# ryanelandt/PressureFieldContact.jl

Measured on AMD Instinct MI355X. Metric: tet-tri clip+integrate ops/s, higher is better.
Workload: dtype f64

## Files before the change

### pressurefieldcontact.jl_amd/csrc/pfc_bp.h

```cpp
#pragma once

struct BpArgs {
    const ItemRec *items;
    const WorkRec *fin;
    WorkRec *fout;
    WorkRec *cand;
    int *fcount;
    int *ccount;
    int *icnt;
    unsigned *status;
    int level, fcap, ccap;
    int n_items;
};

__device__ __forceinline__ void count_per_item(int *icnt, int item, int slot, bool listed, bool flag, int n = 1) {
    if (__ballot(flag) == 0) return;
    const Seg sg = seg_setup(listed ? item : -1);
    const int t = seg_sum(flag ? n : 0, sg);
    if (sg.tail && sg.valid && t != 0) atomicAdd(&icnt[4 * (size_t)item + slot], t);
}

__device__ __forceinline__ NodeRec load_node(const NodeRec *n) {
    union U { vec4i v[9]; NodeRec r; __device__ U() {} } u;
    const gvec4i *p = (const gvec4i *)n;
// ... 185 lines not shown
        if (valid && sub < 9) {
            const int i = sub % 3, jj = sub / 3;
            const double r0 = na->R[3 * i], r1 = na->R[3 * i + 1], r2 = na->R[3 * i + 2];
            T[i + 3 * jj] = (r0 * pose[3 * jj] + r1 * pose[3 * jj + 1]) + r2 * pose[3 * jj + 2];
        } else if (valid && sub < 12) {
            const int i = sub - 9;
            const double r0 = na->R[3 * i], r1 = na->R[3 * i + 1], r2 = na->R[3 * i + 2];
            const double nt = ((-r0) * na->c[0] + (-r1) * na->c[1]) + (-r2) * na->c[2];
            tt[i] = ((r0 * pose[9] + r1 * pose[10]) + r2 * pose[11]) + nt;
        }
        __syncthreads();
        if (valid && sub < 9) {
            const int i = sub % 3, jj = sub / 3;
            const double r = (T[i] * nb->R[3 * jj] + T[i + 3] * nb->R[3 * jj + 1]) + T[i + 6] * nb->R[3 * jj + 2];
            R[i + 3 * jj] = r;
            aR[i + 3 * jj] = __builtin_fabs(r) + 1.0e-14;
        } else if (valid && sub < 12) {
            const int i = sub - 9;
            t[i] = ((T[i] * nb->c[0] + T[i + 3] * nb->c[1]) + T[i + 6] * nb->c[2]) + tt[i];
        }
        __syncthreads();
        bool sep = false;
        if (valid && sub < 15) {
#define EA_(i) (na->e[(i)])
#define EB_(i) (nb->e[(i)])
#define R_(i, j) R[(i) + 3 * (j)]
#define AR_(i, j) aR[(i) + 3 * (j)]
            if (sub < 3) {
                const int i = sub;
                const double rb = (AR_(i, 0) * EB_(0) + AR_(i, 1) * EB_(1)) + AR_(i, 2) * EB_(2);
                sep = (EA_(i) + rb) < __builtin_fabs(t[i]);
            } else if (sub < 6) {
                const int jj = sub - 3;
                const double tl = __builtin_fabs((R_(0, jj) * t[0] + R_(1, jj) * t[1]) + R_(2, jj) * t[2]);
                const double ra = (AR_(0, jj) * EA_(0) + AR_(1, jj) * EA_(1)) + AR_(2, jj) * EA_(2);
                sep = (ra + EB_(jj)) < tl;
            } else {
                const int m = (sub - 6) / 3, jj = (sub - 6) % 3;
                const int u = (m + 1) % 3, v = (m + 2) % 3;
                const int p100 = jj == 0 ? 1 : 0, p221 = jj == 2 ? 1 : 2;
                const double tl = __builtin_fabs(t[v] * R_(u, jj) - t[u] * R_(v, jj));
                const double ra = EA_(u) * AR_(v, jj) + EA_(v) * AR_(u, jj);
                const double rb = EB_(p100) * AR_(m, p221) + EB_(p221) * AR_(m, p100);
                sep = (ra + rb) < tl;
            }
#undef EA_
#undef EB_
#undef R_
#undef AR_
        }
        const unsigned long long ms = __ballot(sep);
        if (valid && sub == 0) und_v[j] = ((ms >> ((tid & 63) & ~15)) & 0xFFFFull) ? 0 : 1;
        __syncthreads();
    }
}


__device__ __forceinline__ int next_ticket_block(int *ctr, int *slot, int n_seed) {
    if ((int)gridDim.x >= n_seed) return n_seed;
    if (threadIdx.x == 0) *slot = (int)gridDim.x + atomicAdd(ctr, 1);
    __syncthreads();
    const int t = *slot;
    __syncthreads();
    return t;
}

template <int BLK>
__device__ __forceinline__ void flush_candidates(const Dfs32Args &g, const int2 *ob, int n_out, int item, int tid,
                                                 int *s_base) {
    if (tid == 0) *s_base = atomicAdd(g.ccount, n_out);
    __syncthreads();
    const int base = *s_base;
    for (int j = tid; j < n_out; j += BLK) {
        if (base + j < g.ccap) {
            WorkRec c;
            c.item = item; c.a = ob[j].x; c.b = ob[j].y; c.pad = 0;
            g.cand[base + j] = c;
        }
    }
    if (tid == 0 && base + n_out > g.ccap) atomicOr(g.status, kStCandOvf);
    __syncthreads();
}

template <int BLK>
__global__ void __launch_bounds__(BLK, 4) k_bp_dfs32(Dfs32Args g) {
    constexpr int kWaves = BLK / 64, kStack = BLK * 10, kOut = BLK * 5;
    __shared__ int2 stk[kStack];
    __shared__ int2 ob[kOut];
    __shared__ int s_cnt[kWaves][2];
    __shared__ int2 und_l[BLK];
    __shared__ int und_v[BLK];
    __shared__ double xs[(BLK / 16) * 33];
    __shared__ int s_seed, s_base, s_def[2];
    __shared__ double s_pose[12];
    __shared__ float s_q12[4];
    __shared__ float s_posef[13];
    __shared__ int s_pose_exact;
    const int tid = threadIdx.x, lane = tid & 63, wave = tid >> 6;
    int n_seed = *g.n_seed;
    if (n_seed > g.seed_cap) n_seed = g.seed_cap;
    const vec4i s_first = ((const gvec4i *)g.seeds)[blockIdx.x];
    for (int sd = blockIdx.x; sd < n_seed; sd = next_ticket_block(g.next_seed, &s_seed, n_seed)) {
        vec4i s_v = s_first;
        if (sd != (int)blockIdx.x) s_v = ((const gvec4i *)g.seeds)[__builtin_amdgcn_readfirstlane(sd)];
        WorkRec s;
        s.item = s_v.x; s.a = s_v.y; s.b = s_v.z; s.pad = s_v.w;
        if ((unsigned)s.item >= (unsigned)g.n_items) {
            if (tid == 0) atomicOr(g.status, kStHole);
            continue;
        }
        const int item = __builtin_amdgcn_readfirstlane(s.item);
        const ItemRec *it = g.items + item;
        if (tid < 9) { const double x = it->R12[tid]; s_pose[tid] = x; s_posef[tid] = (float)x; }
        else if (tid < 12) { const double x = it->t12[tid - 9]; s_pose[tid] = x; s_posef[tid] = (float)x; }
        else if (tid < 16) s_q12[tid - 12] = it->q12[tid - 12];
        else if (tid == 16) s_pose_exact = it->pose_exact;
        else if (tid == 17) s_posef[12] = it->bp_eabs;
        const NodeF *n1 = it->nf1, *n2 = it->nf2;
        int sp = 1, n_out = 0, n_test = 0, n_cand = 0, n_def = 0, n_und = 0;
        if (tid == 0) {
            const int sa = (s.pad & 1) ? ~s.a : s.a;
            const int sb = (s.pad & 2) ? ~s.b : s.b;
            stk[0] = make_int2(sa, sb);
            s_def[0] = s_def[1] = 0;
        }
        __syncthreads();
#ifdef PFC_STAMPS
        unsigned long long c_a = 0, c_b = 0, c_c = 0, c_d = 0, c_it = 0, c_p = 0, c_w1 = 0, c_w2 = 0;
#endif
        int par = 0;
        for (int guard = 0; (sp > 0 || n_def > 0) && guard < (1 << 22); ++guard, par ^= 1) {
            unsigned long long u0 = 0, u1 = 0, u2 = 0, u3 = 0, u4 = 0; (void)u0; (void)u1; (void)u2; (void)u3; (void)u4;
            STAMP(u0);
            const bool settle = n_def > 0;
            int pw = (kStack - g.reserve - sp) / 3;
            int p = sp < BLK ? sp : BLK;
            if (pw < 1) pw = 1;
            if (p > pw) p = pw;
            if (settle) {
                p = n_def;
                exact_pairs_coop<BLK>(it->nodes1, it->nodes2, s_pose, und_l, n_def, xs, und_v, tid);
            }
            const bool act = tid < p;
            int2 e = make_int2(0, 0);
            if (act) e = settle ? und_l[tid] : stk[sp - 1 - tid];
            if (!settle) { sp -= p; n_test += p; } else { n_und += p; }
            int verdict = 0, a0 = 0, a1 = 0, b0 = 0, b1 = 0;
            if (settle && act) verdict = und_v[tid];
            const bool la = act && e.x < 0, lb = act && e.y < 0;
            if (act) {
                const NodeF a = load_nodef(n1 + node_index(e.x));
                const NodeF b = load_nodef(n2 + node_index(e.y));
                a0 = a.link0; a1 = a.link1; b0 = b.link0; b1 = b.link1;
#ifdef PFC_STAMPS
                { float keep = a.e[0] + b.e[0] + a.q[3] + b.q[3]; asm volatile("" ::"v"(keep)); }
                STAMP(u1);
#endif
                if (!settle) {
                    float R12[9], t12[3], q12[4];
#pragma unroll
                    for (int k = 0; k < 9; ++k) R12[k] = s_posef[k];
#pragma unroll
                    for (int k = 0; k < 3; ++k) t12[k] = s_posef[9 + k];
#pragma unroll
                    for (int k = 0; k < 4; ++k) q12[k] = s_q12[k];
                    __builtin_amdgcn_s_setprio(0);
                    verdict = test_pair_f32(a, b, la || lb, R12, q12, t12, s_posef[12]);
                    __builtin_amdgcn_s_setprio(1);
                    if (s_pose_exact) verdict = 2;
                }
            }
            STAMP(u2);
            if (verdict == 2) und_l[atomicAdd(&s_def[par], 1)] = e;
            const bool hit = verdict == 1;
            const bool is_cand = hit && la && lb;
            const bool two = hit && (la != lb);
            const bool four = hit && !la && !lb;
            const unsigned long long mc = __ballot(is_cand), m2 = __ballot(two), m4 = __ballot(four);
            if (lane == 0) {
                s_cnt[wave][0] = __builtin_popcountll(mc);
                s_cnt[wave][1] = 2 * __builtin_popcountll(m2) + 4 * __builtin_popcountll(m4);
            }
#ifdef PFC_STAMPS
            const unsigned long long w1a = __builtin_amdgcn_s_memtime();
#endif
            __syncthreads();
#ifdef PFC_STAMPS
            c_w1 += __builtin_amdgcn_s_memtime() - w1a;
#endif
            STAMP(u3);
            n_def = s_def[par];
            if (tid == 0) s_def[par ^ 1] = 0;
            int c_off = 0, p_off = 0, c_tot = 0, p_tot = 0;
#pragma unroll
            for (int w = 0; w < kWaves; ++w) {
                const int c = s_cnt[w][0], q = s_cnt[w][1];
                if (w < wave) { c_off += c; p_off += q; }
                c_tot += c; p_tot += q;
            }
            if (is_cand) ob[n_out + c_off + prefix_count(mc)] = make_int2(a0, b0);
            if (two | four) {
                const int pos = sp + p_off + 2 * prefix_count(m2) + 4 * prefix_count(m4);
                if (two) {
                    if (la) {
                        stk[pos] = make_int2(e.x, b0); stk[pos + 1] = make_int2(e.x, b1);
                    } else {
                        stk[pos] = make_int2(a0, e.y); stk[pos + 1] = make_int2(a1, e.y);
                    }
                } else {
                    stk[pos] = make_int2(a0, b0); stk[pos + 1] = make_int2(a1, b0);
                    stk[pos + 2] = make_int2(a0, b1); stk[pos + 3] = make_int2(a1, b1);
                }
            }
            n_out += c_tot;
            sp += p_tot;
#ifdef PFC_STAMPS
            const unsigned long long w2a = __builtin_amdgcn_s_memtime();
#endif
            __syncthreads();
#ifdef PFC_STAMPS
            c_w2 += __builtin_amdgcn_s_memtime() - w2a;
#endif
            if (n_out > kOut - BLK || (sp == 0 && n_def == 0 && n_out > 0)) {
                flush_candidates<BLK>(g, ob, n_out, item, tid, &s_base);
                n_cand += n_out;
                n_out = 0;
            }
#ifdef PFC_STAMPS
            STAMP(u4);
            if (!settle) {
                c_a += u1 - u0; c_b += u2 - u1; c_c += u3 - u2; c_d += u4 - u3; c_it += 1; c_p += (unsigned long long)p;
            }
#endif
        }
#ifdef PFC_STAMPS
        if (lane == 0 && g.stamps) { atomicAdd(&g.stamps[0], c_w1); atomicAdd(&g.stamps[1], c_w2); atomicAdd(&g.stamps[2], c_it); }
        if (tid == 0 && g.stamps) {
            atomicAdd(&g.stamps[8], c_a); atomicAdd(&g.stamps[9], c_b); atomicAdd(&g.stamps[10], c_c);
            atomicAdd(&g.stamps[13], c_d); atomicAdd(&g.stamps[11], c_it); atomicAdd(&g.stamps[12], c_p);
        }
#endif
        if (tid == 0) {
            if (sp > 0 || n_def > 0) atomicOr(g.status, kStAbort);
            atomicAdd(&g.icnt[4 * (size_t)item], n_test);
            if (n_cand) atomicAdd(&g.icnt[4 * (size_t)item + 1], n_cand);
            if (n_und) atomicAdd(g.ucount, n_und);
        }
    }
}

struct NodeHead {
    double c[3], e[3];
    int child0, child1, leaf, aabb;
};
__device__ __forceinline__ NodeHead load_head(const NodeRec *n) {
    union { vec4i v[4]; NodeHead h; } u;
    const gvec4i *p = (const gvec4i *)n;
    u.v[0] = p[0]; u.v[1] = p[1]; u.v[2] = p[2]; u.v[3] = p[3];
    return u.h;
}

__global__ void __launch_bounds__(64) k_bp_dfs(DfsArgs g) {
    __shared__ int2 stk[kDfsStack];
    __shared__ int2 ob[kDfsOut];
    const int lane = threadIdx.x;
    int n_seed = *g.n_seed;
    if (n_seed > g.seed_cap) n_seed = g.seed_cap;
    for (int sd = next_ticket(g.next_seed); sd < n_seed; sd = next_ticket(g.next_seed)) {
        const WorkRec s = g.seeds[sd];
        if ((unsigned)s.item >= (unsigned)g.n_items) {
            if (lane == 0) atomicOr(g.status, kStHole);
            continue;
        }
        const int item = __builtin_amdgcn_readfirstlane(s.item);
        const ItemRec *it = g.items + item;
        double R12[9], aR12[9], t12[3];
#pragma unroll
        for (int k = 0; k < 9; ++k) { R12[k] = it->R12[k]; aR12[k] = __builtin_fabs(R12[k]) + 1.0e-14; }
#pragma unroll
        for (int k = 0; k < 3; ++k) t12[k] = it->t12[k];
        const NodeRec *n1 = it->nodes1, *n2 = it->nodes2;
        int sp = 1, n_out = 0, n_test = 0, n_cand = 0;
        if (lane == 0) {
            const int sa = (((const GNodeRec *)n1)[s.a].leaf != kInternal) ? ~s.a : s.a;
            const int sb = (((const GNodeRec *)n2)[s.b].leaf != kInternal) ? ~s.b : s.b;
            stk[0] = make_int2(sa, sb);
        }
        __syncthreads();
#ifdef PFC_STAMPS
        unsigned long long c_load = 0, c_sat = 0, c_push = 0, c_iter = 0, c_lanes = 0;
#endif
        for (int guard = 0; sp > 0 && guard < (1 << 22); ++guard) {
            unsigned long long u0 = 0, u1 = 0, u2 = 0, u3 = 0;
            (void)u0; (void)u1; (void)u2; (void)u3;
            STAMP(u0);
            int pw = (kDfsStack - g.reserve - sp) / 3;
            int p = sp < 64 ? sp : 64;
            if (pw < 1) pw = 1;
            if (p > pw) p = pw;
            const bool act = lane < p;
            int2 e = make_int2(0, 0);
            if (act) e = stk[sp - 1 - lane];
            __syncthreads();
            sp -= p;
            n_test += p;
            const bool la = act && e.x < 0, lb = act && e.y < 0;
            const int ia = node_index(e.x), ib = node_index(e.y);
            NodeHead a, b;
            a.leaf = kInternal; b.leaf = kInternal; a.child0 = a.child1 = b.child0 = b.child1 = 0; a.aabb = b.aabb = 1;
#pragma unroll
            for (int k = 0; k < 3; ++k) { a.c[k] = a.e[k] = b.c[k] = b.e[k] = 0.0; }
            double Ra[9] = {1.0, 0.0, 0.0, 0.0, 1.0, 0.0, 0.0, 0.0, 1.0}, Rb[9] = {1.0, 0.0, 0.0, 0.0, 1.0, 0.0, 0.0, 0.0, 1.0};
            if (act) {
                a = load_head(n1 + ia);
                b = load_head(n2 + ib);
            }
            const bool ra = la || (act && !a.aabb), rb = lb || (act && !b.aabb);
            const bool general = __any(ra || rb);
            if (ra) {
#pragma unroll
                for (int k = 0; k < 9; ++k) Ra[k] = ((const GNodeRec *)n1)[ia].R[k];
            }
// ... 95 lines not shown
```

### pressurefieldcontact.jl_amd/csrc/pfc_hip.hip

```cpp
#include "pfc_kernels.h"

#include <algorithm>
#include <atomic>
#include <chrono>
#include <condition_variable>
#include <functional>
#include <mutex>
#include <thread>
#include <cmath>
#include <cstdlib>
#include <limits>
#include <cstdarg>
#include <cstdio>
#include <cstring>
#include <string>
#include <utility>
#include <vector>

#include "../../include/pfc.h"
#include "pfc_sort.h"

namespace pfc {

__global__ void k_prep_tri(int n, const double *__restrict__ pt, const int *__restrict__ tri, TriRec *__restrict__ out) {
// ... 247 lines not shown
    template <class T> int out(T *host, size_t count) { return add(Out, host, count); }
    template <class T> int scratch(size_t count) { return add(0, (const T *)nullptr, count); }
    hipError_t commit() {
        hipError_t e = nf > kMaxFields ? hipErrorInvalidValue : buf.ensure(total);
        for (int k = 0; k < nf && e == hipSuccess; ++k)
            if ((f[k].dir & In) && f[k].host && f[k].count)
                e = hipMemcpyAsync(buf.p + f[k].off, f[k].host, f[k].elem * f[k].count, hipMemcpyHostToDevice, st);
        return e;
    }
    template <class T> T *at(int k) const { return f[k].host || !f[k].dir ? reinterpret_cast<T *>(buf.p + f[k].off) : nullptr; }
    hipError_t fetch(int k, size_t count) {
        if (!f[k].host || !count) return hipSuccess;
        return hipMemcpyAsync(f[k].host, buf.p + f[k].off, f[k].elem * count, hipMemcpyDeviceToHost, st);
    }
    hipError_t finish() {
        hipError_t e = hipSuccess;
        for (int k = 0; k < nf && e == hipSuccess; ++k)
            if (f[k].dir & Out) e = fetch(k, f[k].count);
        return e == hipSuccess ? hipStreamSynchronize(st) : e;
    }
};

struct KinHost {
    int n_body = 0, nq = 0, nv = 0;
    std::vector<char> blob;
    size_t o_jtype = 0, o_qoff = 0, o_voff = 0, o_path_off = 0, o_path = 0, o_x_p_j = 0, o_axis = 0, o_anc = 0;
    size_t o_sub_off = 0, o_sub = 0, o_inertia = 0;
    bool has_inertia = false;
    double gravity[3] = {0.0, 0.0, 0.0};
    template <class T> size_t put(const std::vector<T> &v) {
        const size_t off = blob.size(), bytes = sizeof(T) * v.size();
        blob.resize((off + bytes + 255) & ~(size_t)255);
        if (bytes) std::memcpy(blob.data() + off, v.data(), bytes);
        return off;
    }
};

struct HostMesh {
    int n_pt = 0, n_tri = 0, n_tet = 0, n_node = 0, n_leaf = 0, depth = 0;
    double Ebar = 0.0;
    std::vector<double> xyz, eps;
    std::vector<int> tri, tet;
    std::vector<NodeRec> nodes;
    std::vector<NodeF> nodesf;
    double cmax = 0.0;
    NodeRec *d_nodes = nullptr;
    NodeF *d_nodesf = nullptr;
    TriRec *d_tri = nullptr;
    TetRec *d_tet = nullptr;
    double *d_tet_eps = nullptr;
};

enum { EV_START = 0, EV_SETUP, EV_BP, EV_NP, EV_BR, EV_FIN, EV_COUNT };

}

struct pfc_multi;
struct pfc_context {
    int device = 0;
    bool finalized = false;
    pfc_multi *multi = nullptr;
    Stream stream;
    Stream twin_stream;
    PinBuf<char, 2> pin_bp;
    int pin_bp_n = 0;
    bool team_owner = false;
    int opt_team_fault = -1;
    int opt_dual_fold = 1;
    int opt_fused_f32 = 1;
    std::string err;
    std::vector<HostMesh> meshes;
    std::vector<InsDev> ins;
    MeshDev *d_meshes = nullptr;
    InsDev *d_ins = nullptr;
    InsFull *d_insfull = nullptr;
    DevBuf<MeshDev> own_meshes;
    DevBuf<InsDev> own_ins;
    DevBuf<InsFull> own_insfull;
    DevBuf<char> mesh_arena;
    int max_levels = 1;
    int max_leaves = 2;
    bool any_bristle = false, any_tet_tet = false;
    int opt_debug = 0, opt_profile = 0, opt_max_levels = 0, opt_bfs_levels = -1, opt_no_filter = 0;
    DevBuf<ItemRec> items;
    DevBuf<WorkRec> frontier[2], cand;
    DevBuf<int> clip_n, icnt, trac_item;
    DevBuf<double> acc, res, trac_d, rec;
    DevBuf<int> ctr;
    DevBuf<unsigned> status;
    DevBuf<unsigned long long> stamps;
    DevBuf<int> tail;
    PinBuf<int> h_tail;
    PinBuf<char, 2> pin_in, pin_out;
    DevBuf<char> bar_in;
    DevBuf<char> bar_din;
    int bar_state = 0;
    PinBuf<char, 2> pin_din, pin_dout;
    long long dual_hint = -1;
    int dual_dev_hyb_skip = 0;
    struct KeptPass {
        enum Kind { None, Batched, HandOver, Hybrid, OneGraph } kind = None;
        int n = 0;
        bool ids = false;
    } kept;
    bool device_kept() const { return kept.kind == KeptPass::Batched || kept.kind == KeptPass::HandOver; }
    struct Pending {
        enum Kind { None, Batched, Fused, More, Surface } kind = None;
        hipStream_t stream = nullptr;
        int split_n0 = 0, n_ctr = 0;
        enum Dual { NoDual, DualBatched, DualHandOver } dual = NoDual;
        int n_dir = 0; size_t dpcap = 0; bool ids = false;
    } pend;
    struct HostPoint {
        int n = 0;
        bool ids = false;
        unsigned long long serial = 0;
        size_t ids_at = 0;
    };
    HostPoint pin_in_pt;
    HostPoint pin_din_pt;
    bool last_dual_reused = false;
    int opt_dual_reuse = 1;
    unsigned long long value_serial = 0;
    std::vector<int> dual_counts_cache;
    DevBuf<double> dual_zero;
    unsigned long long epoch = 0;
    GraphExec gexec[2];
    struct GraphKey {
        int n_items, levels, L, debug, bristle, surv;
        const void *p[9];
        void *stream;
        unsigned long long epoch;
    } gkey[2] = {};
    bool ghave[2] = {false, false};
    GraphExec dgexec;
    struct DualGraphKey { GraphKey v; int n_dir; size_t bound; const void *din, *dout; } dgkey = {};
    bool dghave = false;
    int opt_graph = 1;
    size_t fcap = 0, ccap = 0, tcap = 0, rcap = 0;
    DevBuf<double> h_pose;
    int last_n_items = 0, last_levels = 0, last_bfs_levels = 0;
    long long stats[8] = {0, 0, 0, 0, 0, 0, 0, 0};
    DevBuf<double> dual_in, dual_acc, dual_res, dual_out, dual_poly;
    DevBuf<int2> dual_pkey;
    DevBuf<int> dual_sel, dual_flag;
    DevBuf<char> stage;
    DevBuf<double> sdual_w;
    DevBuf<int> sdual_i;
    DevBuf<char> sdual_tmp;
    DevBuf<int> surv;
    DevBuf<int> rgn;
    DevBuf<int> poly_item, pcnt, poly_cand;
    DevBuf<double> poly;
    long long last_undecided = 0;
    long long last_active = 0;
    struct ShapeHint { int n = 0; bool sparse = false; } hints[4];
    void note_shape(int n, bool sparse) {
        int k = 0;
        while (k < 3 && hints[k].n != n) ++k;
        for (; k > 0; --k) hints[k] = hints[k - 1];
        hints[0].n = n; hints[0].sparse = sparse;
    }
    bool shape_is_sparse(int n) const {
        for (const ShapeHint &e : hints) if (e.n == n) return e.sparse;
        return false;
    }
// ... 236 lines not shown
    if ((e = ensure_graphed(h, h->tail, (size_t)h->max_levels + 40)) != hipSuccess) return e;
    if ((e = h->h_tail.ensure((size_t)h->max_levels + 40)) != hipSuccess) return e;
    if (h->opt_poison) {
        if ((e = hipMemsetAsync(h->frontier[0].p, 0xFF, sizeof(WorkRec) * h->frontier[0].cap, h->stream)) != hipSuccess) return e;
        if ((e = hipMemsetAsync(h->frontier[1].p, 0xFF, sizeof(WorkRec) * h->frontier[1].cap, h->stream)) != hipSuccess) return e;
        if ((e = hipMemsetAsync(h->cand.p, 0xFF, sizeof(WorkRec) * h->cand.cap, h->stream)) != hipSuccess) return e;
        if (h->poly_item.p && (e = hipMemsetAsync(h->poly_item.p, 0xFF, sizeof(int) * h->poly_item.cap, h->stream)) != hipSuccess) return e;
        if ((e = hipStreamSynchronize(h->stream)) != hipSuccess) return e;
    }
    return hipSuccess;
}

TracSoA trac_view(pfc_context *h) {
    TracSoA t;
    size_t n = h->tcap;
    double *d = h->trac_d.p;
    t.item = h->trac_item.p;
    t.nx = d; t.ny = d + n; t.nz = d + 2 * n; t.rx = d + 3 * n; t.ry = d + 4 * n; t.rz = d + 5 * n;
    t.dA = d + 6 * n; t.p = d + 7 * n;
    return t;
}

int eff_levels(const pfc_context *h) {
    return (h->opt_max_levels > 0 && h->opt_max_levels < h->max_levels) ? h->opt_max_levels : h->max_levels;
}

constexpr int kDualSelectMin = 512;
constexpr int kBpSmallBlockMin = 3072;

int bfs_levels_for(const pfc_context *h, int n_items, int levels, bool half) {
    int L = 0;
    if (h->opt_bfs_levels >= 0) {
        L = h->opt_bfs_levels;
    } else {
        const bool big = h->max_leaves >= 8192, mid = h->max_leaves >= 1024;
        const int n_eff = half ? 2 * n_items : n_items;
        const double target = big ? (n_eff >= 600 ? 1.0 : (n_eff >= 256 ? 1024.0 : (n_eff >= 128 ? 2048.0 : (n_eff >= 32 ? 16384.0 : 49152.0))))
                                  : (mid ? 256.0 : 64.0);
        double seeds = (double)n_items;
        while (seeds < target && L < 9) { seeds *= 4.0; ++L; }
    }
    return L > levels ? levels : L;
}

bool pile_mode(const pfc_context *h, int n_items) {
    return h->max_leaves < 8192 && n_items >= 1024 && n_items < kBpSmallBlockMin && h->shape_is_sparse(n_items) && !h->is_twin;
}

int bp_block_for(const pfc_context *h, int n_items, bool half) {
    if (n_items >= kBpSmallBlockMin) return 128;
    if (half) return 256;
    if (h->max_leaves >= 8192 && n_items >= 8 && n_items < 1024) return 512;
    if (pile_mode(h, n_items)) return 512;
    return 256;
}

void launch_broadphase(pfc_context *h, int n_items, int L, bool half, int *ccount, int *fcount, int *next_seed, int *ucount, hipStream_t st) {
    for (int lv = 0; lv < L; ++lv) {
        BpArgs b;
        b.items = h->items.p; b.fin = h->frontier[lv & 1].p; b.fout = h->frontier[(lv + 1) & 1].p;
        b.cand = h->cand.p; b.fcount = fcount; b.ccount = ccount; b.icnt = h->icnt.p; b.status = h->status.p;
        b.level = lv; b.fcap = (int)h->fcap; b.ccap = (int)h->ccap; b.n_items = n_items;
        double ub = (double)n_items * std::pow(4.0, (double)(lv < 15 ? lv : 15));
        size_t bound = ub > (double)h->fcap ? h->fcap : (size_t)ub;
        hipLaunchKernelGGL(k_bp_expand, dim3(grid_for(bound, 256, 2048)), dim3(256), 0, st, b);
    }
    {
        double ub = (double)n_items * std::pow(4.0, (double)(L < 15 ? L : 15));
        size_t bound = ub > (double)h->fcap ? h->fcap : (size_t)ub;
        DfsArgs d;
        d.items = h->items.p; d.cand = h->cand.p; d.ccount = ccount; d.ccap = (int)h->ccap; d.icnt = h->icnt.p;
        d.status = h->status.p; d.reserve = 3 * h->max_levels + 3; d.stamps = h->stamps.p; d.n_items = n_items;
        if (h->opt_no_filter) {
            d.seeds = h->frontier[L & 1].p; d.n_seed = fcount + L; d.seed_cap = (int)h->fcap; d.next_seed = next_seed;
            d.no_filter = 1;
            hipLaunchKernelGGL(k_bp_dfs, dim3(grid_for(bound, 1, 256 * 8)), dim3(64), 0, st, d);
        } else {
            Dfs32Args f;
            f.items = h->items.p; f.seeds = h->frontier[L & 1].p; f.n_seed = fcount + L; f.next_seed = next_seed;
            f.seed_cap = (int)h->fcap; f.cand = h->cand.p; f.ccount = ccount; f.ccap = (int)h->ccap;
            f.ucount = ucount; f.icnt = h->icnt.p; f.status = h->status.p; f.stamps = h->stamps.p;
            f.reserve = 3 * h->max_levels + 3; f.n_items = n_items;
            const int blk = bp_block_for(h, n_items, half);
            if (blk == 128 && f.reserve <= 128 * 10 - 512)
                hipLaunchKernelGGL((k_bp_dfs32<128>), dim3(grid_for(bound, 1, 256 * 8)), dim3(128), 0, st, f);
            else if (blk == 512)
                hipLaunchKernelGGL((k_bp_dfs32<512>), dim3(grid_for(bound, 1, 256 * 2)), dim3(512), 0, st, f);
            else
                hipLaunchKernelGGL((k_bp_dfs32<kDfsBlock>), dim3(grid_for(bound, 1, 256 * 6)), dim3(kDfsBlock), 0, st, f);
        }
    }
}

int record_eval(pfc_context *h, int n_items, const int *d_ins_ids, const double *d_pose, const double *d_twist,
                const double *d_s, double *d_wrench, double *d_sdot, int *d_counts, hipStream_t st, bool prof, const PassOpts &o) {
    new_value_pass(h);
    h->last_dual_reused = false;
    const int levels = eff_levels(h);
    int *ccount = h->ctr.p, *tcount = h->ctr.p + 1, *next_seed = h->ctr.p + 2;
    int *ucount = h->ctr.p + 4, *fcount = h->ctr.p + 6;
    int *pcount = h->ctr.p + ctr_pcount(levels);
#ifdef PFC_STAMPS
    HIP_TRY(h, hipMemsetAsync(h->stamps.p, 0, sizeof(unsigned long long) * 16, st));
#endif
    if (prof) HIP_TRY(h, hipEventRecord(h->ev[EV_START], st));

    EvalArgs ea;
    ea.n_items = n_items; ea.ins_ids = d_ins_ids; ea.pose = d_pose; ea.twist = d_twist; ea.s = d_s;
    ea.bp_pose = o.bp_pose;
    ea.ins = h->d_ins; ea.meshes = h->d_meshes; ea.n_ins = (int)h->ins.size(); ea.items = h->items.p;
    ea.frontier0 = h->frontier[0].p; ea.fcount = fcount; ea.acc = h->acc.p; ea.icnt = h->icnt.p;
    ea.status = h->status.p;
    hipLaunchKernelGGL(k_setup_items, dim3(grid_for(n_items, 64, 1 << 20)), dim3(64), 0, st, ea);
    if (prof) HIP_TRY(h, hipEventRecord(h->ev[EV_SETUP], st));

    const int L = bfs_levels_for(h, n_items, levels, o.half);
    launch_broadphase(h, n_items, L, o.half, ccount, fcount, next_seed, ucount, st);
    if (o.bp_pose)
        hipLaunchKernelGGL(k_repose, dim3(grid_for(n_items, 64, 1 << 20)), dim3(64), 0, st, n_items, d_pose, h->items.p);
    if (h->opt_fixed_order) {
        int ba, bb;
        const int bits = pfc_sort_key_bits(n_items, h->max_elem1, h->max_elem2, &ba, &bb);
        if (bits > 64)
            return fail(h, PFC_ERR_BAD_ARG, "option fixed_order: (item, element, element) needs %d key bits for %d items, more than 64", bits, n_items);
        size_t cover = h->sort_cover ? h->sort_cover : h->ccap;
        if (cover > h->ccap) cover = h->ccap;
        h->sort_cover_used = cover;
        static const bool global_sort = std::getenv("PFC_FIXED_GLOBAL_SORT") != nullptr;
        if (global_sort || h->fixed_whole_list)
            HIP_TRY(h, pfc_sort_candidates(h->cand.p, ccount, cover, h->sort_keys[0].p, h->sort_keys[1].p, h->sort_tmp.p, h->sort_tmp.cap,
                                           n_items, ba, bb, bits, h->status.p, kStFixedCover, st));
        else
            HIP_TRY(h, pfc_canon_candidates(h->cand.p, ccount, cover, h->icnt.p, n_items, h->sort_keys[0].p, h->sort_keys[1].p, h->canon_off.p,
                                            h->canon_fill.p, h->canon_item.p, bb, h->status.p, kStFixedCover, kStFixedBig, st));
        hipLaunchKernelGGL(k_fixed_init, dim3(grid_for(n_items, 256, 1 << 20)), dim3(256), 0, st, n_items, h->det.p);
    }
    if (prof) HIP_TRY(h, hipEventRecord(h->ev[EV_BP], st));

    NpArgs np;
    np.items = h->items.p; np.cand = h->cand.p; np.ccount = ccount; np.ccap = (int)h->ccap; np.acc = h->acc.p;
    np.icnt = h->icnt.p; np.n_items = n_items; np.clip_n = h->opt_debug ? h->clip_n.p : nullptr; np.trac = trac_view(h);
    np.tcount = tcount; np.tcap = (int)h->tcap; np.status = h->status.p; np.debug = h->opt_debug;
    np.stamps = h->stamps.p;
    np.rec = h->rec.p; np.rgn = h->rgn.p; np.rr_cap = (int)(h->rcap / kRgn);
    np.poly_item = h->poly_item.p; np.poly = h->poly.p; np.pcap = (int)poly_cap(h->ccap);
    np.pcnt = h->pcnt.p; np.chunk_switch = kNpChunkSwitch; np.poly_cand = o.list ? h->poly_cand.p : nullptr;
    np.surv = o.list ? h->surv.p : nullptr; np.scount = pcount + 1;
    const int np_grid = grid_for(h->ccap, kNpBlock, kNpMaxBlocks);
    int bin_split = 0;
    np.bin_split = 0;
    const int np_mode = h->opt_debug ? 1 : ((h->opt_fixed_order || (h->opt_clip_min > 0 && n_items >= h->opt_clip_min)) ? 2 : 0);
    if (np_mode == 1) {
        if (h->any_tet_tet) hipLaunchKernelGGL((k_narrow<true, 1>), dim3(np_grid), dim3(kNpBlock), 0, st, np);
        else hipLaunchKernelGGL((k_narrow<false, 1>), dim3(np_grid), dim3(kNpBlock), 0, st, np);
    } else if (np_mode == 0) {
        if (h->any_tet_tet) hipLaunchKernelGGL((k_narrow<true, 0>), dim3(np_grid), dim3(kNpBlock), 0, st, np);
        else hipLaunchKernelGGL((k_narrow<false, 0>), dim3(np_grid), dim3(kNpBlock), 0, st, np);
    } else {
        if (h->opt_clip_queue && !h->any_tet_tet) {
            if (!o.list && !h->opt_fixed_order) bin_split = h->opt_bin_split;
            np.bin_split = bin_split;
            hipLaunchKernelGGL(k_clip_queue, dim3(np_grid), dim3(kNpBlock), 0, st, np);
        } else if (o.half || (n_items >= 640 && n_items < 1024)) {
            if (h->any_tet_tet) hipLaunchKernelGGL((k_narrow<true, 3>), dim3(np_grid), dim3(kNpBlock), 0, st, np);
            else hipLaunchKernelGGL((k_narrow<false, 3>), dim3(np_grid), dim3(kNpBlock), 0, st, np);
        } else {
            if (h->any_tet_tet) hipLaunchKernelGGL((k_narrow<true, 2>), dim3(np_grid), dim3(kNpBlock), 0, st, np);
            else hipLaunchKernelGGL((k_narrow<false, 2>), dim3(np_grid), dim3(kNpBlock), 0, st, np);
        }
        IntegArgs ig;
        ig.items = h->items.p; ig.n_items = n_items; ig.ccount = ccount; ig.ccap = (int)h->ccap; ig.chunk_switch = kNpChunkSwitch;
        ig.pcnt = h->pcnt.p; ig.bin_split = bin_split; ig.poly_item = h->poly_item.p; ig.poly = h->poly.p; ig.pcap = np.pcap;
// ... 742 lines not shown
            if (e1 > h->max_elem1) h->max_elem1 = e1;
            if (m2.n_tet > h->max_elem2) h->max_elem2 = m2.n_tet;
        }
        int lv = h->meshes[in.m1].depth + h->meshes[in.m2].depth + 1;
        if (lv > h->max_levels) h->max_levels = lv;
        const int lf = h->meshes[in.m1].n_leaf + h->meshes[in.m2].n_leaf;
        if (lf > h->max_leaves) h->max_leaves = lf;
        if (in.model == PFC_BRISTLE) h->any_bristle = true;
        if (h->meshes[in.m1].n_tri == 0) h->any_tet_tet = true;
    }
    if (3 * h->max_levels + 3 > kDfsStack - 128 || 3 * h->max_levels + 3 > kDfsStack32 - 1024)
        return fail(h, PFC_ERR_BAD_ARG, "OBB trees too deep (depth sum %d): rebuild them balanced", h->max_levels - 1);
    if (!h->ins.empty()) {
        HIP_TRY(h, h->own_ins.ensure(h->ins.size()));
        h->d_ins = h->own_ins.p;
        HIP_TRY(h, copy_sync(h, h->d_ins, h->ins.data(), sizeof(InsDev) * h->ins.size(), hipMemcpyHostToDevice));
        std::vector<InsFull> full(h->ins.size());
        for (size_t k = 0; k < h->ins.size(); ++k) {
            const InsDev &in = h->ins[k];
            const HostMesh &m1 = h->meshes[in.m1], &m2 = h->meshes[in.m2];
            InsFull f;
            std::memset(&f, 0, sizeof f);
            f.nodes1 = m1.d_nodes; f.nodes2 = m2.d_nodes; f.nf1 = m1.d_nodesf; f.nf2 = m2.d_nodesf;
            f.tri = m1.d_tri; f.tet = m2.d_tet; f.tet1 = m1.d_tri ? nullptr : m1.d_tet; f.eps1 = m1.d_tet_eps; f.eps2 = m2.d_tet_eps;
            f.chi = in.chi; f.Ebar = m2.Ebar; f.Ebar1 = m1.Ebar; f.mu_s = in.mu_s; f.mu_d = in.mu_d; f.v_c = in.v_c;
            f.tau = in.tau; f.k_bar = in.k_bar; f.magic = in.magic;
            f.model = in.model; f.nq = in.nq; f.n_node1 = m1.n_node; f.n_node2 = m2.n_node;
            f.reserve = 3 * (m1.depth + m2.depth + 1) + 3;
            f.cmax12 = m1.cmax + m2.cmax;
            full[k] = f;
        }
        HIP_TRY(h, h->own_insfull.ensure(full.size()));
        h->d_insfull = h->own_insfull.p;
        HIP_TRY(h, copy_sync(h, h->d_insfull, full.data(), sizeof(InsFull) * full.size(), hipMemcpyHostToDevice));
    }
    h->finalized = true;
    return PFC_OK;
}

static int check_eval_args(pfc_context *h, int n_items, const void *ins_ids, const void *pose, const void *twist,
                           const void *s, const void *wrench, const void *sdot) {
    if (!h->finalized) return fail(h, PFC_ERR_STATE, "pfc_eval before pfc_finalize");
    if (n_items < 0) return fail(h, PFC_ERR_BAD_ARG, "negative n_items");
    if (n_items == 0) return PFC_OK;
    if (h->ins.empty()) return fail(h, PFC_ERR_STATE, "no contact instructions");
    if (!pose || !twist || !wrench || !sdot) return fail(h, PFC_ERR_BAD_ARG, "null buffer");
    if (!ins_ids && n_items > (int)h->ins.size())
        return fail(h, PFC_ERR_BAD_ARG, "n_items exceeds the number of instructions and no ins_ids given");
    if (h->any_bristle && !s) return fail(h, PFC_ERR_BAD_ARG, "bristle instructions need the state buffer s");
    return PFC_OK;
}

static int eval_device(pfc_context *h, int n_items, const int *d_ins_ids, const double *d_pose, const double *d_twist,
                       const double *d_s, double *d_wrench, double *d_sdot, int *d_counts, void *stream, PassOpts o) {
    { const int rc = check_eval_args(h, n_items, d_ins_ids, d_pose, d_twist, d_s, d_wrench, d_sdot); if (rc != PFC_OK) return rc; }
    drop_pending(h);
    end_kept_pass(h);
    if (n_items == 0) { h->last_n_items = 0; return PFC_OK; }
    HIP_TRY(h, hipSetDevice(h->device));
    hipStream_t st = stream ? (hipStream_t)stream : h->stream;
    int team = fused_team(h, n_items, o);
    if (team > 1 && !team_acquire(h)) team = fused_ok(h, n_items, o) ? 1 : 0;
    if (team) {
        o.nw = team;
        const int rc_t = enqueue_fused(h, n_items, d_ins_ids, d_pose, d_twist, d_s, d_wrench, d_sdot, d_counts, st, o);
        if (rc_t != PFC_OK) team_release(h);
        return rc_t;
    }
    if (h->fused_skip > 0 && n_items <= kFusedMaxItems) --h->fused_skip;
    const bool split = h->opt_split_min > 0 && n_items >= h->opt_split_min && d_ins_ids && !h->opt_debug && !h->opt_fixed_order &&
                       !o.list && !h->is_twin && !pile_mode(h, n_items);
    if (!split) return enqueue_eval(h, n_items, d_ins_ids, d_pose, d_twist, d_s, d_wrench, d_sdot, d_counts, st, o);
    int rc = make_twin(h);
    if (rc != PFC_OK) return rc;
    pfc_context *t = h->twin;
    t->opt_profile = h->opt_profile; t->opt_max_levels = h->opt_max_levels; t->opt_bfs_levels = h->opt_bfs_levels;
    t->opt_poison = h->opt_poison;
    if (t->opt_clip_min != h->opt_clip_min) { t->opt_clip_min = h->opt_clip_min; t->ghave[0] = t->ghave[1] = false; }
    if (t->opt_clip_queue != h->opt_clip_queue) { t->opt_clip_queue = h->opt_clip_queue; t->ghave[0] = t->ghave[1] = false; }
    if (t->opt_bin_split != h->opt_bin_split) { t->opt_bin_split = h->opt_bin_split; t->ghave[0] = t->ghave[1] = false; }
    if (t->opt_vertex_fields != h->opt_vertex_fields) { t->opt_vertex_fields = h->opt_vertex_fields; t->ghave[0] = t->ghave[1] = false; }
    t->opt_graph = h->opt_graph;
    if (t->opt_no_filter != h->opt_no_filter) { t->opt_no_filter = h->opt_no_filter; t->ghave[0] = t->ghave[1] = false; }
    const int n0 = n_items / 2, n1 = n_items - n0;
    hipStream_t s0 = h->stream;
    HIP_TRY(h, hipEventRecord(h->ev_fork, st));
    if (s0 != st) HIP_TRY(h, hipStreamWaitEvent(s0, h->ev_fork, 0));
    HIP_TRY(h, hipStreamWaitEvent(t->stream, h->ev_fork, 0));
    o.half = true;
    rc = enqueue_eval(h, n0, d_ins_ids, d_pose, d_twist, d_s, d_wrench, d_sdot, d_counts, s0, o);
    if (rc != PFC_OK) return rc;
    if (o.bp_pose) o.bp_pose += 24 * (size_t)n0;
    o.tail = nullptr;
    rc = enqueue_eval(t, n1, d_ins_ids + n0, d_pose + 24 * (size_t)n0, d_twist + 6 * (size_t)n0,
                      d_s ? d_s + 6 * (size_t)n0 : nullptr, d_wrench + 6 * (size_t)n0, d_sdot + 6 * (size_t)n0,
                      d_counts ? d_counts + 4 * (size_t)n0 : nullptr, t->stream, o);
    if (rc != PFC_OK) { h->err = t->err; return rc; }
    HIP_TRY(h, hipEventRecord(h->ev_join, t->stream));
    HIP_TRY(h, hipStreamWaitEvent(st, h->ev_join, 0));
    if (s0 != st) {
        HIP_TRY(h, hipEventRecord(h->ev_join0, s0));
        HIP_TRY(h, hipStreamWaitEvent(st, h->ev_join0, 0));
    }
    h->pend = {pfc_context::Pending::Batched, s0, n0};
    return PFC_OK;
}

int pfc_eval_device(pfc_handle h, int n_items, const int *d_ins_ids, const double *d_pose, const double *d_twist,
                    const double *d_s, double *d_wrench, double *d_sdot, int *d_counts, void *stream) {
    if (!h) return PFC_ERR_BAD_ARG;
    if (h->multi)
        return multi_eval_device(h, n_items, 0, d_ins_ids, d_pose, nullptr, d_twist, d_s, nullptr, nullptr, nullptr, d_wrench, d_sdot,
                                 nullptr, nullptr, d_counts, stream);
    return eval_device(h, n_items, d_ins_ids, d_pose, d_twist, d_s, d_wrench, d_sdot, d_counts, stream, PassOpts());
}

namespace {

struct SurfFricOut {
    const double *s;
    double *fric, *fric_summary, *stiff;
};

int surface_enqueue(pfc_context *h, int n_items, const int *d_ins_ids, const double *d_pose, const double *d_twist, long long cap_poly,
                    long long cap_trac, long long *d_poly_off, int *d_poly_idx, double *d_poly_xyz, long long *d_poly_trac,
                    double *d_trac, double *d_summary, int *d_counts, long long *d_totals, hipStream_t st, const SurfFricOut *fo = nullptr) {
    new_value_pass(h);
    drop_pending(h);
    h->pin_in_pt = {}; h->pin_din_pt = {};
    int ba, bb;
    const int bits = pfc_sort_key_bits(n_items, h->max_elem1, h->max_elem2, &ba, &bb);
    if (bits > 64)
        return fail(h, PFC_ERR_BAD_ARG, "pfc_contact_surface: (item, element, element) needs %d key bits for %d items, more than 64", bits, n_items);
    HIP_TRY(h, ensure_work(h, n_items, false));
    const size_t c = h->ccap;
    HIP_TRY(h, h->surf_cnt.ensure(2 * (c + 1)));
    HIP_TRY(h, h->surf_off.ensure(2 * (c + 1)));
    HIP_TRY(h, h->surf_part.ensure(c * kSurfSums));
    HIP_TRY(h, h->surf_seg.ensure((size_t)n_items + 1));
    HIP_TRY(h, h->surf_canon_off.ensure((size_t)n_items + 1));
    HIP_TRY(h, h->surf_canon_fill.ensure((size_t)n_items));
    HIP_TRY(h, h->surf_canon_item.ensure(c));
    HIP_TRY(h, h->surf_keys[0].ensure(c));
    HIP_TRY(h, h->surf_keys[1].ensure(c));
    if (fo) {
        HIP_TRY(h, h->sfric_mom.ensure((size_t)n_items * kFricSplit * kFricMom));
        HIP_TRY(h, h->sfric_sum.ensure((size_t)n_items * kFricSplit * kFricSums));
        HIP_TRY(h, h->sfric_res.ensure((size_t)n_items * kResStride));
    }
    size_t scan_bytes = 0, sort_bytes = 0;
    HIP_TRY(h, pfc_scan_pairs(nullptr, &scan_bytes, nullptr, nullptr, c + 1, st));
    if (h->surf_whole_list) HIP_TRY(h, pfc_sort_temp_bytes(c, bits, &sort_bytes));
    HIP_TRY(h, h->surf_tmp.ensure((scan_bytes > sort_bytes ? scan_bytes : sort_bytes) + 16));
    const int levels = eff_levels(h);
    const int n_ctr = levels + 12;
    HIP_TRY(h, h->surf_out.ensure((size_t)n_ctr + 3));
    HIP_TRY(h, h->h_surf.ensure((size_t)n_ctr + 3));
    int *ccount = h->ctr.p, *next_seed = h->ctr.p + 2, *ucount = h->ctr.p + 4, *fcount = h->ctr.p + 6;

    EvalArgs ea;
    ea.n_items = n_items; ea.ins_ids = d_ins_ids; ea.pose = d_pose; ea.twist = d_twist; ea.s = fo ? fo->s : nullptr; ea.bp_pose = nullptr;
    ea.ins = h->d_ins; ea.meshes = h->d_meshes; ea.n_ins = (int)h->ins.size(); ea.items = h->items.p;
    ea.frontier0 = h->frontier[0].p; ea.fcount = fcount; ea.acc = h->acc.p; ea.icnt = h->icnt.p;
    ea.status = h->status.p;
    hipLaunchKernelGGL(k_setup_items, dim3(grid_for(n_items, 64, 1 << 20)), dim3(64), 0, st, ea);
    const int L = bfs_levels_for(h, n_items, levels, false);
// ... 2116 lines not shown
        copy_out_dual(po + n * 12, nk, d_wrench, d_sdot);
        h->dual_counts_cache.assign(pc, pc + n * 4);
        h->pin_din_pt = {n_items, ins_ids != nullptr, h->value_serial, in_d};
        return PFC_OK;
    }
    o.list = true;
    int rc = eval_host(h, n_items, ins_ids, pose, twist, s, wrench, sdot, counts, o);
    if (rc != PFC_OK) return rc;
    HIP_TRY(h, ensure_graphed(h, h->dual_in, nk * 36));
    HIP_TRY(h, ensure_graphed(h, h->dual_acc, nk * kDaStride));
    HIP_TRY(h, ensure_graphed(h, h->dual_res, nk * kDrStride));
    HIP_TRY(h, ensure_graphed(h, h->dual_out, nk * 12));
    double *dp = h->dual_in.p, *dt = dp + nk * 24, *dsd = dt + nk * 6;
    const size_t in_bytes = sizeof(double) * nk * 36, out_bytes = sizeof(double) * nk * 12;
    HIP_TRY(h, h->pin_in.ensure(in_bytes));
    HIP_TRY(h, h->pin_out.ensure(out_bytes));
    pack_seeds((double *)h->pin_in.p, nk, d_pose, d_twist, d_s, true);
    HIP_TRY(h, hipMemcpyAsync(dp, h->pin_in.p, in_bytes, hipMemcpyHostToDevice, st));
    rc = launch_dual(h, n_items, n_dir, h->tail.p, dp, dt, dsd, h->dual_out.p, h->dual_out.p + nk * 6, (size_t)h->stats[2], st, nullptr);
    if (rc != PFC_OK) return rc;
    h->dual_hint = h->stats[2];
    HIP_TRY(h, hipMemcpyAsync(h->pin_out.p, h->dual_out.p, out_bytes, hipMemcpyDeviceToHost, st));
    HIP_TRY(h, hipStreamSynchronize(st));
    copy_out_dual((const double *)h->pin_out.p, nk, d_wrench, d_sdot);
    return PFC_OK;
}

int pfc_eval_dual(pfc_handle h, int n_items, int n_dir, const int *ins_ids, const double *pose, const double *twist,
                  const double *s, const double *d_pose, const double *d_twist, const double *d_s, double *wrench,
                  double *sdot, double *d_wrench, double *d_sdot, int *counts) {
    return pfc_eval_dual_bp(h, n_items, n_dir, ins_ids, pose, nullptr, twist, s, d_pose, d_twist, d_s, wrench, sdot, d_wrench, d_sdot, counts);
}

int pfc_set_option(pfc_handle h, const char *name, long long value) {
    if (!h || !name) return PFC_ERR_BAD_ARG;
    if (h->multi) {
        if (!std::strcmp(name, "multi_min")) { h->multi->opt_min_items = value < 1 ? 1 : (int)value; h->multi->part_n = 0; return PFC_OK; }
        h->multi->dev_kept = false;
        for (pfc_context *c : h->multi->shard) {
            const int rc = on_shard(h, c, [&](pfc_context *c1) { return pfc_set_option(c1, name, value); });
            if (rc != PFC_OK) return rc;
        }
        return PFC_OK;
    }
    end_kept_pass(h);
    if (!std::strcmp(name, "debug")) h->opt_debug = value != 0;
    else if (!std::strcmp(name, "profile")) h->opt_profile = value != 0;
    else if (!std::strcmp(name, "max_levels")) {
        if (value < 0 || value > (1 << 20) || (h->finalized && value > h->max_levels))
            return fail(h, PFC_ERR_BAD_ARG, "max_levels must be 0 (automatic) or 1..%d (depth of the finalized trees + 1)", h->max_levels);
        h->opt_max_levels = (int)value; h->ghave[0] = h->ghave[1] = false; h->dghave = false;
    }
    else if (!std::strcmp(name, "bfs_levels")) h->opt_bfs_levels = (int)value;
    else if (!std::strcmp(name, "graph")) h->opt_graph = value != 0;
    else if (!std::strcmp(name, "split_min")) h->opt_split_min = (int)value;
    else if (!std::strcmp(name, "dual_reuse")) h->opt_dual_reuse = (int)value;
    else if (!std::strcmp(name, "clip_min")) { h->opt_clip_min = (int)value; h->ghave[0] = h->ghave[1] = false; h->dghave = false; }
    else if (!std::strcmp(name, "clip_queue")) { h->opt_clip_queue = (int)value; h->ghave[0] = h->ghave[1] = false; h->dghave = false; }
    else if (!std::strcmp(name, "vertex_fields")) {
        if (value != 0 && value != 1) return fail(h, PFC_ERR_BAD_ARG, "vertex_fields must be 0 (per-point k_fric) or 1 (per-corner fields)");
        h->opt_vertex_fields = (int)value; h->ghave[0] = h->ghave[1] = false; h->dghave = false;
    }
    else if (!std::strcmp(name, "bin_split")) {
        const long long sp = value < 0 ? -value : value;
        if (value != 0 && (sp < 3 || sp > 9))
            return fail(h, PFC_ERR_BAD_ARG, "bin_split must be 0 (dense fill), 3..9 (polygons of fewer vertices fill a 512-candidate chunk from its front) or -9..-3 (chunks of every size)");
        h->opt_bin_split = (int)value; h->ghave[0] = h->ghave[1] = false; h->dghave = false;
    }
    else if (!std::strcmp(name, "poison")) h->opt_poison = value != 0;
    else if (!std::strcmp(name, "fused")) { h->opt_fused = value != 0; h->fused_skip = 0; }
    else if (!std::strcmp(name, "team")) h->opt_team = value < 0 ? 0 : (value > kTeamMaxWg ? kTeamMaxWg : (int)value);
    else if (!std::strcmp(name, "team_fault")) h->opt_team_fault = (int)value;
    else if (!std::strcmp(name, "fused_f32")) h->opt_fused_f32 = value != 0;
    else if (!std::strcmp(name, "dual_fold")) { h->opt_dual_fold = value != 0; h->dghave = false; }
    else if (!std::strcmp(name, "fixed_order")) {
        const int on = value != 0;
        if (on != h->opt_fixed_order) {
            h->opt_fixed_order = on; h->fused_skip = 0;
            h->ghave[0] = h->ghave[1] = false; h->dghave = false;
            h->rec.release();
        }
    }
    else if (!std::strcmp(name, "no_filter")) { h->opt_no_filter = (int)value; h->ghave[0] = h->ghave[1] = false; h->dghave = false; }
    else return fail(h, PFC_ERR_BAD_ARG, "unknown option %s", name);
    return PFC_OK;
}

int pfc_get_stats(pfc_handle h, long long *out8) {
    if (!h || !out8) return PFC_ERR_BAD_ARG;
    if (h->multi) { for (int k = 0; k < 8; ++k) out8[k] = h->multi->stats[k]; return PFC_OK; }
    for (int k = 0; k < 8; ++k) out8[k] = h->stats[k];
    return PFC_OK;
}

int pfc_get_stage_ms(pfc_handle h, float *out6) {
    if (!h || !out6) return PFC_ERR_BAD_ARG;
    if (h->multi)
        return on_first_shard(h, [&](pfc_context *c) { return pfc_get_stage_ms(c, out6); });
    if (!h->ev_valid) return fail(h, PFC_ERR_STATE, "profile option was off for the last evaluation");
    HIP_TRY(h, hipSetDevice(h->device));
    HIP_TRY(h, hipEventSynchronize(h->ev[EV_FIN]));
    for (int k = 0; k < 5; ++k) HIP_TRY(h, hipEventElapsedTime(&out6[k], h->ev[k], h->ev[k + 1]));
    HIP_TRY(h, hipEventElapsedTime(&out6[5], h->ev[EV_START], h->ev[EV_FIN]));
    if (h->last_parts == 2 && h->twin && h->twin->ev_valid) {
        pfc_context *t = h->twin;
        float b[6];
        HIP_TRY(h, hipEventSynchronize(t->ev[EV_FIN]));
        for (int k = 0; k < 5; ++k) HIP_TRY(h, hipEventElapsedTime(&b[k], t->ev[k], t->ev[k + 1]));
        HIP_TRY(h, hipEventElapsedTime(&b[5], t->ev[EV_START], t->ev[EV_FIN]));
        for (int k = 0; k < 5; ++k) out6[k] = 0.5f * (out6[k] + b[k]);
        if (b[5] > out6[5]) out6[5] = b[5];
    }
    return PFC_OK;
}

int pfc_last_parts(pfc_handle h) { return h ? (h->multi ? pfc_last_parts(h->multi->shard[0]) : (h->last_fused ? 0 : h->last_parts)) : 0; }
int pfc_last_team(pfc_handle h) { return h ? (h->multi ? pfc_last_team(h->multi->shard[0]) : (h->last_fused ? h->last_fu_nw : 0)) : 0; }
int pfc_last_dual_reused(pfc_handle h) {
    if (!h) return 0;
    if (h->multi) {
        for (int k = 0; k < h->multi->n_used; ++k)
            if (h->multi->bound[k + 1] > h->multi->bound[k] && !h->multi->shard[k]->last_dual_reused) return 0;
        return 1;
    }
    return h->last_dual_reused ? 1 : 0;
}

int pfc_debug_pairs(pfc_handle h, int item, int *pairs, int *clip_n, int cap) {
    if (!h) return -PFC_ERR_BAD_ARG;
    if (h->multi) {
        int local = 0;
        pfc_context *c = multi_locate(h, item, &local);
        if (!c) return -fail(h, PFC_ERR_BAD_ARG, "bad item");
        return on_shard(h, c, [&](pfc_context *c1) { return pfc_debug_pairs(c1, local, pairs, clip_n, cap); }, true);
    }
    if (!h->opt_debug) return -fail(h, PFC_ERR_STATE, "debug option is off");
    { int rc = drain(h); if (rc) return -rc; }
    if (item < 0 || item >= h->last_n_items) return -fail(h, PFC_ERR_BAD_ARG, "bad item");
    size_t nc = (size_t)h->stats[1];
    std::vector<WorkRec> c(nc);
    std::vector<int> cn(nc);
    if (nc) {
        if (copy_sync(h, c.data(), h->cand.p, sizeof(WorkRec) * nc, hipMemcpyDeviceToHost) != hipSuccess ||
            copy_sync(h, cn.data(), h->clip_n.p, sizeof(int) * nc, hipMemcpyDeviceToHost) != hipSuccess)
            return -fail(h, PFC_ERR_HIP, "copy failed");
    }
    int n = 0;
    for (size_t k = 0; k < nc; ++k)
        if (c[k].item == item) {
            if (n < cap) {
                if (pairs) { pairs[2 * n] = c[k].a; pairs[2 * n + 1] = c[k].b; }
                if (clip_n) clip_n[n] = cn[k];
            }
            ++n;
        }
    return n;
}

int pfc_debug_tractions(pfc_handle h, int item, double *buf, int cap) {
    if (!h) return -PFC_ERR_BAD_ARG;
    if (h->multi) {
        int local = 0;
        pfc_context *c = multi_locate(h, item, &local);
        if (!c) return -fail(h, PFC_ERR_BAD_ARG, "bad item");
        return on_shard(h, c, [&](pfc_context *c1) { return pfc_debug_tractions(c1, local, buf, cap); }, true);
    }
// ... 821 lines not shown
```

Baseline: 4.145 billion.

## Batch deferred exact pair tests in broad-phase DFS instead of settling each iteration

Adds a DEFER template mode to the broad-phase DFS kernel. Pairs needing exact f64 testing now accumulate and are settled cooperatively only when the stack is empty, the batch reaches half a block, or stack room runs low. Overflow beyond BLK is pushed back onto the DFS stack. This aims to amortise the cost of the cooperative exact-test iteration, which otherwise runs for only a few pairs at a time, but it raises stack pressure and adds extra bookkeeping. Extra stamp counters are also added for profiling.

```diff
diff --git a/pressurefieldcontact.jl_amd/csrc/pfc_bp.h b/pressurefieldcontact.jl_amd/csrc/pfc_bp.h
--- a/pressurefieldcontact.jl_amd/csrc/pfc_bp.h
+++ b/pressurefieldcontact.jl_amd/csrc/pfc_bp.h
@@ -291,7 +291,7 @@
     __syncthreads();
 }
 
-template <int BLK>
+template <int BLK, bool DEFER>
 __global__ void __launch_bounds__(BLK, 4) k_bp_dfs32(Dfs32Args g) {
     constexpr int kWaves = BLK / 64, kStack = BLK * 10, kOut = BLK * 5;
     __shared__ int2 stk[kStack];
@@ -300,7 +300,7 @@
     __shared__ int2 und_l[BLK];
     __shared__ int und_v[BLK];
     __shared__ double xs[(BLK / 16) * 33];
-    __shared__ int s_seed, s_base, s_def[2];
+    __shared__ int s_seed, s_base, s_def;
     __shared__ double s_pose[12];
     __shared__ float s_q12[4];
     __shared__ float s_posef[13];
@@ -320,34 +320,41 @@
         }
         const int item = __builtin_amdgcn_readfirstlane(s.item);
         const ItemRec *it = g.items + item;
-        if (tid < 9) { const double x = it->R12[tid]; s_pose[tid] = x; s_posef[tid] = (float)x; }
-        else if (tid < 12) { const double x = it->t12[tid - 9]; s_pose[tid] = x; s_posef[tid] = (float)x; }
-        else if (tid < 16) s_q12[tid - 12] = it->q12[tid - 12];
-        else if (tid == 16) s_pose_exact = it->pose_exact;
-        else if (tid == 17) s_posef[12] = it->bp_eabs;
+        int ts = tid;
+        asm volatile("" : "+v"(ts));
+        if (ts < 9) { const double x = it->R12[ts]; s_pose[ts] = x; s_posef[ts] = (float)x; }
+        else if (ts < 12) { const double x = it->t12[ts - 9]; s_pose[ts] = x; s_posef[ts] = (float)x; }
+        else if (ts < 16) s_q12[ts - 12] = it->q12[ts - 12];
+        else if (ts == 16) s_pose_exact = it->pose_exact;
+        else if (ts == 17) s_posef[12] = it->bp_eabs;
         const NodeF *n1 = it->nf1, *n2 = it->nf2;
         int sp = 1, n_out = 0, n_test = 0, n_cand = 0, n_def = 0, n_und = 0;
         if (tid == 0) {
             const int sa = (s.pad & 1) ? ~s.a : s.a;
             const int sb = (s.pad & 2) ? ~s.b : s.b;
             stk[0] = make_int2(sa, sb);
-            s_def[0] = s_def[1] = 0;
+            s_def = 0;
         }
         __syncthreads();
 #ifdef PFC_STAMPS
         unsigned long long c_a = 0, c_b = 0, c_c = 0, c_d = 0, c_it = 0, c_p = 0, c_w1 = 0, c_w2 = 0;
-#endif
-        int par = 0;
-        for (int guard = 0; (sp > 0 || n_def > 0) && guard < (1 << 22); ++guard, par ^= 1) {
-            unsigned long long u0 = 0, u1 = 0, u2 = 0, u3 = 0, u4 = 0; (void)u0; (void)u1; (void)u2; (void)u3; (void)u4;
+        unsigned long long c_sit = 0, c_sc = 0, c_sp = 0, c_nc = 0;
+        unsigned long long c_back = 0;
+#endif
+        for (int guard = 0; (sp > 0 || n_def > 0) && guard < (1 << 22); ++guard) {
+            unsigned long long u0 = 0, u1 = 0, u2 = 0, u3 = 0, u4 = 0, u5 = 0; (void)u0; (void)u1; (void)u2; (void)u3; (void)u4; (void)u5;
             STAMP(u0);
-            const bool settle = n_def > 0;
-            int pw = (kStack - g.reserve - sp) / 3;
-            int p = sp < BLK ? sp : BLK;
-            if (pw < 1) pw = 1;
-            if (p > pw) p = pw;
-            if (settle) {
+            const int room = kStack - g.reserve - sp - 4 * n_def;
+            const bool settle = n_def > 0 && (!DEFER || sp == 0 || n_def >= BLK / 2 || room < 3);
+            int p;
+            if (!settle) {
+                int pw = room / 3;
+                p = sp < BLK ? sp : BLK;
+                if (pw < 1) pw = 1;
+                if (p > pw) p = pw;
+            } else {
                 p = n_def;
+                if (tid == 0) s_def = 0;
                 exact_pairs_coop<BLK>(it->nodes1, it->nodes2, s_pose, und_l, n_def, xs, und_v, tid);
             }
             const bool act = tid < p;
@@ -380,7 +387,11 @@
                 }
             }
             STAMP(u2);
-            if (verdict == 2) und_l[atomicAdd(&s_def[par], 1)] = e;
+            int park = -1;
+            if (verdict == 2) {
+                park = atomicAdd(&s_def, 1);
+                if (!DEFER || park < BLK) und_l[park] = e;
+            }
             const bool hit = verdict == 1;
             const bool is_cand = hit && la && lb;
             const bool two = hit && (la != lb);
@@ -398,8 +409,9 @@
             c_w1 += __builtin_amdgcn_s_memtime() - w1a;
 #endif
             STAMP(u3);
-            n_def = s_def[par];
-            if (tid == 0) s_def[par ^ 1] = 0;
+            n_def = s_def;
+            int n_back = 0;
+            if (DEFER && n_def > BLK) { n_back = n_def - BLK; n_def = BLK; }
             int c_off = 0, p_off = 0, c_tot = 0, p_tot = 0;
 #pragma unroll
             for (int w = 0; w < kWaves; ++w) {
@@ -421,14 +433,19 @@
                     stk[pos + 2] = make_int2(a0, b1); stk[pos + 3] = make_int2(a1, b1);
                 }
             }
+            if (DEFER && park >= BLK) stk[sp + p_tot + (park - BLK)] = e;
             n_out += c_tot;
-            sp += p_tot;
+            sp += p_tot + n_back;
+            n_test -= n_back;
 #ifdef PFC_STAMPS
             const unsigned long long w2a = __builtin_amdgcn_s_memtime();
 #endif
             __syncthreads();
 #ifdef PFC_STAMPS
             c_w2 += __builtin_amdgcn_s_memtime() - w2a;
+            STAMP(u5);
+            if (settle) { c_sit += 1; c_sc += u5 - u0; c_sp += (unsigned long long)p; } else { c_nc += u5 - u0; }
+            c_back += (unsigned long long)n_back;
 #endif
             if (n_out > kOut - BLK || (sp == 0 && n_def == 0 && n_out > 0)) {
                 flush_candidates<BLK>(g, ob, n_out, item, tid, &s_base);
@@ -447,6 +464,8 @@
         if (tid == 0 && g.stamps) {
             atomicAdd(&g.stamps[8], c_a); atomicAdd(&g.stamps[9], c_b); atomicAdd(&g.stamps[10], c_c);
             atomicAdd(&g.stamps[13], c_d); atomicAdd(&g.stamps[11], c_it); atomicAdd(&g.stamps[12], c_p);
+            atomicAdd(&g.stamps[3], c_sit); atomicAdd(&g.stamps[4], c_sc); atomicAdd(&g.stamps[6], c_sp); atomicAdd(&g.stamps[15], c_nc);
+            atomicAdd(&g.stamps[14], c_back);
         }
 #endif
         if (tid == 0) {
diff --git a/pressurefieldcontact.jl_amd/csrc/pfc_hip.hip b/pressurefieldcontact.jl_amd/csrc/pfc_hip.hip
--- a/pressurefieldcontact.jl_amd/csrc/pfc_hip.hip
+++ b/pressurefieldcontact.jl_amd/csrc/pfc_hip.hip
@@ -353,6 +353,7 @@
     int max_leaves = 2;
     bool any_bristle = false, any_tet_tet = false;
     int opt_debug = 0, opt_profile = 0, opt_max_levels = 0, opt_bfs_levels = -1, opt_no_filter = 0;
+    int opt_bp_defer = 1;
     DevBuf<ItemRec> items;
     DevBuf<WorkRec> frontier[2], cand;
     DevBuf<int> clip_n, icnt, trac_item;
@@ -755,12 +756,20 @@
             f.ucount = ucount; f.icnt = h->icnt.p; f.status = h->status.p; f.stamps = h->stamps.p;
             f.reserve = 3 * h->max_levels + 3; f.n_items = n_items;
             const int blk = bp_block_for(h, n_items, half);
-            if (blk == 128 && f.reserve <= 128 * 10 - 512)
-                hipLaunchKernelGGL((k_bp_dfs32<128>), dim3(grid_for(bound, 1, 256 * 8)), dim3(128), 0, st, f);
-            else if (blk == 512)
-                hipLaunchKernelGGL((k_bp_dfs32<512>), dim3(grid_for(bound, 1, 256 * 2)), dim3(512), 0, st, f);
-            else
-                hipLaunchKernelGGL((k_bp_dfs32<kDfsBlock>), dim3(grid_for(bound, 1, 256 * 6)), dim3(kDfsBlock), 0, st, f);
+            const bool defer = h->opt_bp_defer != 0 && !pile_mode(h, n_items);
+            if (blk == 128 && f.reserve <= 128 * 10 - 512) {
+                const dim3 grid(grid_for(bound, 1, 256 * 8));
+                if (defer) hipLaunchKernelGGL((k_bp_dfs32<128, true>), grid, dim3(128), 0, st, f);
+                else hipLaunchKernelGGL((k_bp_dfs32<128, false>), grid, dim3(128), 0, st, f);
+            } else if (blk == 512) {
+                const dim3 grid(grid_for(bound, 1, 256 * 2));
+                if (defer) hipLaunchKernelGGL((k_bp_dfs32<512, true>), grid, dim3(512), 0, st, f);
+                else hipLaunchKernelGGL((k_bp_dfs32<512, false>), grid, dim3(512), 0, st, f);
+            } else {
+                const dim3 grid(grid_for(bound, 1, 256 * 6));
+                if (defer) hipLaunchKernelGGL((k_bp_dfs32<kDfsBlock, true>), grid, dim3(kDfsBlock), 0, st, f);
+                else hipLaunchKernelGGL((k_bp_dfs32<kDfsBlock, false>), grid, dim3(kDfsBlock), 0, st, f);
+            }
         }
     }
 }
@@ -1669,6 +1678,7 @@
     if (t->opt_vertex_fields != h->opt_vertex_fields) { t->opt_vertex_fields = h->opt_vertex_fields; t->ghave[0] = t->ghave[1] = false; }
     t->opt_graph = h->opt_graph;
     if (t->opt_no_filter != h->opt_no_filter) { t->opt_no_filter = h->opt_no_filter; t->ghave[0] = t->ghave[1] = false; }
+    if (t->opt_bp_defer != h->opt_bp_defer) { t->opt_bp_defer = h->opt_bp_defer; t->ghave[0] = t->ghave[1] = false; }
     const int n0 = n_items / 2, n1 = n_items - n0;
     hipStream_t s0 = h->stream;
     HIP_TRY(h, hipEventRecord(h->ev_fork, st));
@@ -3951,6 +3961,10 @@
         }
     }
     else if (!std::strcmp(name, "no_filter")) { h->opt_no_filter = (int)value; h->ghave[0] = h->ghave[1] = false; h->dghave = false; }
+    else if (!std::strcmp(name, "bp_defer")) {
+        if (value != 0 && value != 1) return fail(h, PFC_ERR_BAD_ARG, "bp_defer must be 0 (settle a parked pair in the next iteration) or 1 (in batches)");
+        h->opt_bp_defer = (int)value; h->ghave[0] = h->ghave[1] = false; h->dghave = false;
+    }
     else return fail(h, PFC_ERR_BAD_ARG, "unknown option %s", name);
     return PFC_OK;
 }
```

New measurement: 4.184 billion, median of 6. About the same (+0.9%).
